# jmg049/Spectrograms

Measured on AMD Instinct MI355X. Metric: STFT frames/sec (f32, n_fft=1024 hop=256), higher is better.
Workload: dtype f32

## Files before the change

### spectrograms_amd/csrc/kernels_r32x16.hip

```cpp
#include <type_traits>
#include <utility>

#include "binaural_kind.h"
#include "buffer_ops.h"
#include "fft_inreg.h"
#include "r32x16_layout.h"
#include "sgx_internal.h"

namespace sgx {
namespace {

using namespace inreg;
using namespace r32x16;

typedef int v4i __attribute__((ext_vector_type(4)));
typedef int v2i __attribute__((ext_vector_type(2)));

__device__ __forceinline__ float db_f32(float x) { return __builtin_log2f(x) * 3.01029995663981195f; }

template <int AMP>
__device__ __forceinline__ float amp_f32(float p, float eps) {
    if constexpr (AMP == AMP_MAGNITUDE) return sqrtf(p);
    else if constexpr (AMP == AMP_DB) return db_f32(fmaxf(p, eps));
    else return p;
// ... 36 lines not shown
#ifndef SGX_ODDHOP
#define SGX_ODDHOP 1
#endif
#ifndef SGX_DMA
#define SGX_DMA 0
#endif
#ifndef SGX_ONEPATH
#define SGX_ONEPATH 1
#endif

template <int OFF>
__device__ __forceinline__ void ds_read64(v2f &d, unsigned addr) {
    asm volatile("ds_read_b64 %0, %1 offset:%2" : "=v"(d) : "v"(addr), "n"(OFF));
}
template <int OFF>
__device__ __forceinline__ void ds_read128(v4f &d, unsigned addr) {
    asm volatile("ds_read_b128 %0, %1 offset:%2" : "=v"(d) : "v"(addr), "n"(OFF));
}
template <int N>
__device__ __forceinline__ void tie8(v2f *d) {
    if constexpr (N >= 0)
        asm volatile("s_waitcnt lgkmcnt(%8)"
                     : "+v"(d[0]), "+v"(d[1]), "+v"(d[2]), "+v"(d[3]), "+v"(d[4]), "+v"(d[5]), "+v"(d[6]), "+v"(d[7])
                     : "n"(N));
    else
        asm volatile("" : "+v"(d[0]), "+v"(d[1]), "+v"(d[2]), "+v"(d[3]), "+v"(d[4]), "+v"(d[5]), "+v"(d[6]), "+v"(d[7]));
}
template <int N>
__device__ __forceinline__ void tie16(v2f (&d)[16]) {
    tie8<N>(&d[0]);
    tie8<-1>(&d[8]);
}
template <bool XSPAD, int N1>
constexpr int col_off() { return N1 * 128 + (XSPAD ? (N1 >> 3) * 128 : 0); }
template <bool XSPAD, int PAR, int... K>
__device__ __forceinline__ void read_cols(v2f (&x)[16], v2f (&w)[16], unsigned xaddr, unsigned waddr, std::integer_sequence<int, K...>) {
    ((ds_read64<col_off<XSPAD, 2 * K + PAR>()>(x[K], xaddr), ds_read64<(2 * K + PAR) * 128>(w[K], waddr)), ...);
}

template <int HOP>
constexpr int p512_off_a(int n1) { return 64 * n1 + (64 * n1 / (8 * HOP)) * 64; }
template <int HOP>
constexpr int p512_off_b(int n1) { return 64 * n1 + 4 * HOP + ((64 * n1 + 4 * HOP) / (8 * HOP)) * 64; }
template <int O0, int O1>
__device__ __forceinline__ void ds_read2x32(v2f &d, unsigned addr) {
    static_assert(O0 >= 0 && O0 < 256 && O1 >= 0 && O1 < 256, "ds_read2_b32: 8-bit dword offsets");
    asm volatile("ds_read2_b32 %0, %1 offset0:%2 offset1:%3" : "=v"(d) : "v"(addr), "n"(O0), "n"(O1));
}
template <int HOP, int PAR, int... K>
__device__ __forceinline__ void read_cols512(v2f (&x)[16], v2f (&w)[16], const unsigned (&base)[8], unsigned waddr, std::integer_sequence<int, K...>) {
    ((ds_read2x32<(p512_off_a<HOP>(2 * K + PAR) - p512_off_a<HOP>((2 * K + PAR) & ~3)) / 4, (p512_off_b<HOP>(2 * K + PAR) - p512_off_a<HOP>((2 * K + PAR) & ~3)) / 4>(
          x[K], base[(2 * K + PAR) >> 2]),
      ds_read64<(2 * K + PAR) * 128>(w[K], waddr)),
     ...);
}

template <int PAR, int... K>
__device__ __forceinline__ void read_cols_odd(v2f (&x)[16], v2f (&w)[16], const unsigned (&base)[4], unsigned waddr, std::integer_sequence<int, K...>) {
    ((ds_read2x32<((2 * K + PAR) & 7) * 32, ((2 * K + PAR) & 7) * 32 + 1>(x[K], base[(2 * K + PAR) >> 3]), ds_read64<(2 * K + PAR) * 128>(w[K], waddr)), ...);
}

template <int PAR, int... K>
__device__ __forceinline__ void read_win(v2f (&w)[16], unsigned waddr, std::integer_sequence<int, K...>) {
    (ds_read64<(2 * K + PAR) * 128>(w[K], waddr), ...);
}

template <int OFF>
__device__ __forceinline__ void dma16_to_lds(__amdgpu_buffer_rsrc_t r, int voff, unsigned lds_base) {
    unsigned keep;
    asm volatile("s_mov_b32 %0, m0\n\ts_mov_b32 m0, %3\n\ts_nop 0\n\tbuffer_load_dwordx4 %1, %2, 0 offen offset:%4 lds\n\ts_mov_b32 m0, %0"
                 : "=&s"(keep)
                 : "v"(voff), "s"(r), "s"(lds_base), "n"(OFF)
                 : "memory");
}
template <bool XSPAD, int R, int ROUNDS>
__device__ __forceinline__ void dma_rounds(__amdgpu_buffer_rsrc_t r, int voff, unsigned xs_base, unsigned wave) {
    if constexpr (R < ROUNDS) {
        const unsigned c0 = R * 256u + wave * 64u;
        dma16_to_lds<0>(r, voff + R * 4096, xs_base + c0 * 16u + (XSPAD ? (c0 >> 6) * 128u : 0u));
        dma_rounds<XSPAD, R + 1, ROUNDS>(r, voff, xs_base, wave);
    }
}

__device__ __forceinline__ void load_tw1(const StftArgs &a, unsigned n2, v2f (&twa)[4], v2f (&twb)[8]) {
    const v2f *t1 = (const v2f *)a.tw1 + n2;
#pragma unroll
    for (int q = 0; q < 4; ++q) twa[q] = t1[16 * 8 * q];
#pragma unroll
    for (int q = 0; q < 8; ++q) twb[q] = t1[16 * q];
}

__device__ __forceinline__ void twiddle_store(v2f (&xr)[32], const v2f (&twa)[4], const v2f (&twb)[8], unsigned char *dst) {
#pragma unroll
    for (int k1 = 0; k1 < 32; ++k1) {
        const int qa = k1 >> 3, qb = k1 & 7;
        v2f r = xr[k1];
        if (qb) r = cmulv(r, twb[qb]);
        if (qa) r = cmulv(r, twa[qa]);
#if defined(SGX_ABL_NOEXW)
        asm volatile("" ::"v"(r), "v"(dst));
#elif defined(SGX_ABL_ADDTID)
        asm volatile("ds_write_addtid_b32 %0 offset:%2\n\tds_write_addtid_b32 %1 offset:%3" ::"v"(r.x), "v"(r.y), "n"(k1 * 512), "n"(k1 * 512 + 256) : "memory");
#else
        *(v2f *)(dst + k1 * 128) = r;
#endif
    }
}

__device__ __forceinline__ void read_rows(const unsigned char *exf, unsigned ra, unsigned rb, v2f (&A)[16], v2f (&B)[16]) {
    const v4f *pa = (const v4f *)(exf + ra * 128);
    const v4f *pb = (const v4f *)(exf + rb * 128);
#pragma unroll
    for (int c = 0; c < 8; ++c) {
        const v4f q = pa[c];
        A[2 * c] = (v2f){q.x, q.y};
        A[2 * c + 1] = (v2f){q.z, q.w};
    }
#pragma unroll
    for (int c = 0; c < 8; ++c) {
        const v4f q = pb[c];
        B[2 * c] = (v2f){q.x, q.y};
        B[2 * c + 1] = (v2f){q.z, q.w};
    }
}

struct JobOfs {
    unsigned a1, b1, a2, b2, mid;
};
__device__ __forceinline__ JobOfs job_offsets(unsigned j, unsigned n_frames) {
    const unsigned c1 = j == 0 ? 16u : j, c2 = j == 0 ? 0u : j + 256u;
    return JobOfs{c1 * n_frames, (512u - 224u - c1) * n_frames, c2 * n_frames, (512u - 224u - c2) * n_frames, 256u * n_frames};
}

struct PwAddr {
    float *up, *down;
};
template <int MODE, int AMP, bool PWT>
__device__ __forceinline__ void pass2_compute(v2f (&A)[16], v2f (&B)[16], bool j0, float eps, const v4f *tw, __amdgpu_buffer_rsrc_t ro,
                                              unsigned oa1, unsigned ob1, unsigned oa2, unsigned ob2, unsigned omid, unsigned step,
                                              float *pw_c1, float *pw_m1, float *pw_c2, float *pw_m2, float *pw_mid SGX_STAMP_PARAMS) {
    Fft<16, false>::run(A, A);
    Fft<16, false>::run(B, B);
    const v2f a8 = A[8];
    if (j0) {
        v2f nA[16], nB[8];
#pragma unroll
        for (int i = 0; i < 8; ++i) { nA[i] = B[i]; nA[8 + i] = A[i]; }
        nB[7] = A[0];
#pragma unroll
        for (int t = 1; t < 8; ++t) nB[7 - t] = A[16 - t];
#pragma unroll
        for (int i = 0; i < 16; ++i) A[i] = nA[i];
#pragma unroll
        for (int i = 0; i < 8; ++i) B[i] = nB[i];
        asm volatile("" ::: "memory");
    }
    SGX_STAMP(9);
    constexpr int PSTEP = MODE == OUT_BINAURAL ? 32 * 16 * 2 : PWT ? 32 * 16 : 32;
    auto emit = [&](unsigned voff, unsigned soff, float *pwp, v2f X, bool conj) {
#ifdef SGX_ABL_NOSTORE
        asm volatile("" ::"v"(X), "v"(voff));
        return;
#endif
        if constexpr (MODE == OUT_COMPLEX) {
            const v2f V = conj ? (v2f){X.x, -X.y} : X;
            __builtin_amdgcn_raw_buffer_store_b64(__builtin_bit_cast(v2i, V), ro, (int)voff, (int)soff, 0);
        } else if constexpr (MODE == OUT_MEL) {
#ifdef SGX_ABL_NOPW
            asm volatile("" ::"v"(X), "v"(pwp));
            return;
#endif
            *pwp = AMP == AMP_MAG_IN ? sqrtf(power_of(X)) : power_of(X);
        } else if constexpr (MODE == OUT_BINAURAL) {
            *(v2f *)pwp = conj ? (v2f){X.x, -X.y} : X;
        } else {
            __builtin_amdgcn_raw_buffer_store_b32(__builtin_bit_cast(int, amp_f32<AMP>(power_of(X), eps)), ro, (int)voff, (int)soff, 0);
        }
    };
    auto split = [&](v2f P, v2f Q, v4f w, v2f &X, v2f &Y) {
        const v2f E = pfma(Q, (v2f){1.f, -1.f}, P);
        const v2f D = pfma(Q, (v2f){-1.f, 1.f}, P);
        const v2f T = pfma(hi2(D), (v2f){w.z, w.w}, lo2(D) * (v2f){w.x, w.y});
        X = E + T;
        Y = E - T;
    };
#pragma unroll
    for (int i = 0; i < 8; ++i) {
        v2f X, Y;
        split(A[i], B[15 - i], tw[i], X, Y);
        emit(oa1, i * step, pw_c1 + i * PSTEP, X, false);
        emit(ob1, (7 - i) * step, pw_m1 + (7 - i) * PSTEP, Y, true);
    }
#pragma unroll
    for (int t = 0; t < 8; ++t) {
        v2f X, Y;
        split(A[8 + t], B[7 - t], tw[8 + t], X, Y);
        emit(oa2, t * step, pw_c2 + t * PSTEP, X, false);
        emit(ob2, (7 - t) * step, pw_m2 + (7 - t) * PSTEP, Y, true);
    }
    if (j0) emit(omid, 0u, pw_mid, a8 * (v2f){2.f, -2.f}, false);
    SGX_STAMP(10);
}

constexpr unsigned kP512Step = 16u * 64u;
template <int MODE, int AMP, bool PACK = false>
__device__ __forceinline__ void pass2_pair512(v2f (&A)[16], v2f (&B)[16], bool j0, float eps, __amdgpu_buffer_rsrc_t ro, unsigned vfull1,
                                              unsigned vhalf1, unsigned vfull2, unsigned vhalf2, unsigned vfullm, unsigned vhalfm, unsigned step,
                                              float *pw1, float *pw2, float *pwm) {
    Fft<16, false>::run(A, A);
    Fft<16, false>::run(B, B);
    const v2f a8 = A[8];
    if (j0) {
        v2f nA[16], nB[8];
#pragma unroll
        for (int i = 0; i < 8; ++i) { nA[i] = B[i]; nA[8 + i] = A[i]; }
        nB[7] = A[0];
#pragma unroll
        for (int t = 1; t < 8; ++t) nB[7 - t] = A[16 - t];
#pragma unroll
        for (int i = 0; i < 16; ++i) A[i] = nA[i];
#pragma unroll
        for (int i = 0; i < 8; ++i) B[i] = nB[i];
        asm volatile("" ::: "memory");
    }
    auto emit = [&](unsigned vfull, unsigned vhalf, int soff, v2f Xa, v2f Xb, bool conj, float *pwp) {
        if constexpr (MODE == OUT_MEL) {
            const float pa = power_of(Xa), pb = power_of(Xb);
            *(v2f *)pwp = AMP == AMP_MAG_IN ? (v2f){sqrtf(pa), sqrtf(pb)} : (v2f){pa, pb};
        } else if constexpr (MODE == OUT_COMPLEX) {
            const float sg = conj ? -1.f : 1.f;
            const v4f V = (v4f){Xa.x, sg * Xa.y, Xb.x, sg * Xb.y};
            if constexpr (PACK) {
                __builtin_amdgcn_raw_buffer_store_b64(__builtin_bit_cast(v2i, (v2f){V.x, V.y}), ro, (int)vfull, soff, 0);
                __builtin_amdgcn_raw_buffer_store_b64(__builtin_bit_cast(v2i, (v2f){V.z, V.w}), ro, (int)vhalf, soff, 0);
            } else {
                __builtin_amdgcn_raw_buffer_store_b128(__builtin_bit_cast(v4i, V), ro, (int)vfull + soff, 0, 0);
                __builtin_amdgcn_raw_buffer_store_b64(__builtin_bit_cast(v2i, (v2f){V.x, V.y}), ro, (int)vhalf, soff, 0);
            }
        } else {
            const v2f V = (v2f){amp_f32<AMP>(power_of(Xa), eps), amp_f32<AMP>(power_of(Xb), eps)};
            if constexpr (PACK) {
                const float va = V.x, vb = V.y;
                __builtin_amdgcn_raw_buffer_store_b32(__builtin_bit_cast(int, va), ro, (int)vfull, soff, 0);
                __builtin_amdgcn_raw_buffer_store_b32(__builtin_bit_cast(int, vb), ro, (int)vhalf, soff, 0);
            } else {
                __builtin_amdgcn_raw_buffer_store_b64(__builtin_bit_cast(v2i, V), ro, (int)vfull, soff, 0);
                __builtin_amdgcn_raw_buffer_store_b32(__builtin_bit_cast(int, V.x), ro, (int)vhalf, soff, 0);
            }
        }
    };
    auto pair = [&](v2f P, v2f Q, v2f &Xa, v2f &Xb) {
        Xa = pfma(Q, (v2f){1.f, -1.f}, P);
        const v2f D = pfma(Q, (v2f){-1.f, 1.f}, P);
        Xb = (v2f){D.y, -D.x};
    };
#pragma unroll
    for (int i = 0; i < 8; ++i) {
        v2f Xa, Xb;
        pair(A[i], B[15 - i], Xa, Xb);
        emit(vfull1, vhalf1, i * (int)step, Xa, Xb, false, pw1 + i * kP512Step);
    }
#pragma unroll
    for (int t = 0; t < 8; ++t) {
        v2f Xa, Xb;
        pair(A[8 + t], B[7 - t], Xa, Xb);
        if (j0) emit(vfull2 + t * step, vhalf2 + t * step, 0, Xa, Xb, false, pw2 + t * kP512Step);
        else emit(vfull2 + (7 - t) * step, vhalf2 + (7 - t) * step, 0, Xa, Xb, true, pw2 + (7 - t) * kP512Step);
    }
    if (j0) emit(vfullm, vhalfm, 0, (v2f){2.f * a8.x, 0.f}, (v2f){2.f * a8.y, 0.f}, false, pwm);
}

template <int AMP>
__device__ __forceinline__ void mel_tile_csr(const StftArgs &a, const float *pwall, unsigned b, unsigned f0, unsigned nf,
                                             float eps, unsigned t, unsigned nthreads) {
    const float *val = (const float *)a.mel_val;
    float *o = (float *)a.out + ((size_t)b * a.n_out) * a.n_frames + f0;
    for (unsigned idx = t; idx < 16u * a.n_mels; idx += nthreads) {
        const unsigned ff = idx & 15u, mm = idx >> 4;
        float acc = 0.0f;
// ... 277 lines not shown
__device__ __forceinline__ void mel_tile_sched512(const StftArgs &a, const float *pwT, const unsigned *sched, unsigned b, unsigned f0,
                                                  unsigned nf, float eps, unsigned tid) {
    const unsigned wave = __builtin_amdgcn_readfirstlane(tid >> 6), lane = tid & 63u, slot = lane >> 4, fp = lane & 15u;
    const unsigned obytes = (a.n_out * a.n_frames - f0) * 4u;
    const __amdgpu_buffer_rsrc_t ro = make_rsrc((const float *)a.out + (size_t)b * a.n_out * a.n_frames + f0, obytes);
    constexpr unsigned kDrop = 0x80000000u;
    const unsigned fo0 = 2u * fp < nf ? 8u * fp : kDrop, fo1 = 2u * fp + 1u < nf ? 8u * fp + 4u : kDrop;
    const uint4 *info = (const uint4 *)(sched + kSchedHdr) + wave * 8u + slot;
    uint4 ca = info[0], cb = info[4];
#pragma unroll
    for (unsigned seg = 0; seg < (unsigned)kSchedSegs; ++seg) {
        const uint4 na = info[(seg + 1u) * 32u], nb = info[(seg + 1u) * 32u + 4u];
        const unsigned L = __builtin_amdgcn_readfirstlane(ca.x);
        const v4f *wa = (const v4f *)((const float *)sched + ca.y), *wb = (const v4f *)((const float *)sched + cb.y);
        const v4f *pa = (const v4f *)(pwT + (ca.z >> 1) * 64u) + fp, *pb = (const v4f *)(pwT + (cb.z >> 1) * 64u) + fp;
        v2f acca = {0.0f, 0.0f}, accb = {0.0f, 0.0f};
        for (unsigned t = 0; t < L; t += 4u) {
            const v4f w4a = wa[t >> 2], a0 = pa[(t >> 1) * 16u], a1 = pa[(t >> 1) * 16u + 16u];
            const v4f w4b = wb[t >> 2], b0 = pb[(t >> 1) * 16u], b1 = pb[(t >> 1) * 16u + 16u];
            acca = mul_add_unfused(w4a.x, (v2f){a0.x, a0.y}, acca);
            accb = mul_add_unfused(w4b.x, (v2f){b0.x, b0.y}, accb);
            acca = mul_add_unfused(w4a.y, (v2f){a0.z, a0.w}, acca);
            accb = mul_add_unfused(w4b.y, (v2f){b0.z, b0.w}, accb);
            acca = mul_add_unfused(w4a.z, (v2f){a1.x, a1.y}, acca);
            accb = mul_add_unfused(w4b.z, (v2f){b1.x, b1.y}, accb);
            acca = mul_add_unfused(w4a.w, (v2f){a1.z, a1.w}, acca);
            accb = mul_add_unfused(w4b.w, (v2f){b1.z, b1.w}, accb);
        }
        const bool ha = ca.w != 0xffffffffu, hb = cb.w != 0xffffffffu;
        const unsigned boa = ca.w * a.n_frames * 4u, bob = cb.w * a.n_frames * 4u;
        __builtin_amdgcn_raw_buffer_store_b32(__builtin_bit_cast(int, amp_f32<AMP>(acca.x, eps)), ro, (int)((ha && fo0 != kDrop) ? boa + fo0 : kDrop), 0, 0);
        __builtin_amdgcn_raw_buffer_store_b32(__builtin_bit_cast(int, amp_f32<AMP>(acca.y, eps)), ro, (int)((ha && fo1 != kDrop) ? boa + fo1 : kDrop), 0, 0);
        __builtin_amdgcn_raw_buffer_store_b32(__builtin_bit_cast(int, amp_f32<AMP>(accb.x, eps)), ro, (int)((hb && fo0 != kDrop) ? bob + fo0 : kDrop), 0, 0);
        __builtin_amdgcn_raw_buffer_store_b32(__builtin_bit_cast(int, amp_f32<AMP>(accb.y, eps)), ro, (int)((hb && fo1 != kDrop) ? bob + fo1 : kDrop), 0, 0);
        ca = na;
        cb = nb;
    }
}

template <int KIND>
__device__ __forceinline__ void binaural_tile(const StftArgs &a, const unsigned char *smem_all, unsigned b, unsigned f0, unsigned nf) {
    binaural::KindConst<float> c;
    c.pi = 3.14159265358979323846f;
    c.two_pi = 2.0f * c.pi;
    c.bw = (float)a.bin_bw;
    c.power = a.bin_power;
    c.wrapped = a.bin_wrapped;
    const v2f *L = (const v2f *)smem_all, *R = (const v2f *)(smem_all + kExBytes);
    float *out = (float *)a.out + ((size_t)b * a.bin_count) * a.n_frames + f0;
    for (unsigned i = threadIdx.x; i < a.bin_count * 16u; i += 512u) {
        const unsigned r = i >> 4, f = i & 15u, k = a.bin_start + r;
        const v2f l = L[k * 16u + f], q = R[k * 16u + f];
        const float v = binaural::binaural_value<float, KIND>(l.x, l.y, q.x, q.y, k, c);
        if (f < nf) out[(size_t)r * a.n_frames + f] = v;
    }
}

template <int MODE, int AMP, int ROUNDS, bool WIDE, bool XSPAD, bool PWT, int HOP512 = 0, bool PACK = false, int MSTEPS = 0>
__global__ __launch_bounds__(512, 2) void k_r32x16(StftArgs a, unsigned per_xcd, unsigned total, unsigned slots) {
    constexpr bool MFCC = MSTEPS != 0;
    static_assert(!MFCC || (PWT && AMP == AMP_DB && HOP512 == 0 && !PACK), "fused MFCC epilogue: Mel-dB on the schedule, n_fft 1024, one-signal tiles");
    constexpr bool P512 = HOP512 != 0;
    constexpr bool BIN = MODE == OUT_BINAURAL;
    static_assert(!BIN || (!WIDE && !PWT && !P512 && !PACK && !MFCC), "binaural: one-signal n_fft 1024 tiles, per-half pass 2");
    constexpr unsigned HS = BIN ? 1u : 2u;
    static_assert(!PACK || (ROUNDS == 0 && !WIDE && !XSPAD && (HOP512 == 0 ? (MODE != OUT_MEL || PWT) : MODE != OUT_MEL)),
                  "PACK: direct loads, one-half tiles; n_fft 1024: scheduled band stage, n_fft 512: per-bin outputs");
    constexpr unsigned SS512 = 8u * HOP512;
    static_assert(!P512 || PACK || (HOP512 % 4 == 0 && ROUNDS * 256 * 4 >= 31 * HOP512 + 512), "P512: 16-byte chunks, the whole tile staged");
    static_assert(!WIDE || MODE != OUT_MEL, "wide pass 2 needs a per-bin output");
    static_assert(!PWT || MODE == OUT_MEL, "PWT is a filterbank layout");
    static_assert(!P512 || (!WIDE && !XSPAD && (ROUNDS > 0 || PACK) && (PWT == (MODE == OUT_MEL))), "P512: staged samples (PACK: per-lane loads), scheduled band stage");
    constexpr bool DMA = SGX_DMA != 0 && PWT && ROUNDS > 0 && !P512;
    constexpr unsigned FPT = P512 ? 32u : 16u;
    constexpr unsigned NB = P512 ? 257u : 513u;
    extern __shared__ __attribute__((aligned(16))) unsigned char smem_all[];
    const unsigned half = __builtin_amdgcn_readfirstlane(threadIdx.x >> 8);
    const unsigned tid = threadIdx.x & 255u;
    constexpr bool H256M = HOP512 == 256 && MODE == OUT_MEL && !PACK;
    constexpr unsigned EXB = H256M ? (unsigned)kExBytesH256 : (unsigned)kExBytes, POFF = H256M ? (unsigned)kOutOffH256 : (unsigned)kOutOff;
    unsigned char *smem = smem_all + half * EXB;
    unsigned char *tabs = smem_all + 2 * EXB;
    if (threadIdx.x < 256u) ((v4f *)(tabs + kWinOff))[threadIdx.x] = ((const v4f *)a.window)[threadIdx.x];
    for (unsigned i = threadIdx.x; i < 16u * 17u; i += 512u) ((v4f *)(tabs + kTw2Off))[i] = ((const v4f *)a.tw2)[i];
    unsigned *sched = (unsigned *)(tabs + kMelOff);
    if constexpr (PWT)
        for (unsigned i = threadIdx.x; i < a.mel_sched_words; i += 512u) sched[i] = a.mel_sched[i];
    float *mfrag = (float *)(tabs + kMelOff) + ((a.mel_sched_words + 3u) & ~3u);
    if constexpr (MFCC)
        for (unsigned i = threadIdx.x; i < a.mfcc_frag_words; i += 512u) mfrag[i] = ((const float *)a.mfcc_frag)[i];

    const unsigned xcd = blockIdx.x & 7u, slot = blockIdx.x >> 3;
    const unsigned lo = xcd * per_xcd;
    const unsigned hi = min(lo + per_xcd, total);
    unsigned wid = lo + slot * HS + (BIN ? 0u : half);
    unsigned lead = lo + slot * HS;

    const unsigned p1f = tid >> 4, n2 = tid & 15u;
    const unsigned lane = tid & 63u;
    const unsigned wv_ = WIDE ? threadIdx.x >> 6 : tid >> 6;
    const unsigned jq = WIDE ? lane >> 5 : lane >> 4, p2f = WIDE ? lane & 31u : lane & 15u;
    const unsigned j = wv_ + (WIDE ? 8u : 4u) * jq;
    const unsigned ra = j, rb = j == 0 ? 16u : 32u - j;
    const float eps = (float)a.eps;
    constexpr unsigned ES = MODE == OUT_COMPLEX ? 8u : 4u;
    const JobOfs jo = job_offsets(j, a.n_frames);
    const unsigned step = 32u * a.n_frames * ES;
    const v4f *twj = (const v4f *)(tabs + kTw2Off) + j * 17u;
    v2f twa[4], twb[8];
    load_tw1(a, n2, twa, twb);

    constexpr int NCR = ROUNDS > 0 ? ROUNDS : 1;
    v4f creg[NCR];
    v2f xd[ROUNDS > 0 ? 1 : 32];
    const unsigned chunks = XSPAD ? 1216u : P512 ? (31u * HOP512 + 512u + 3u) >> 2 : (15u * a.hop + 1024u + 3u) >> 2;
    const unsigned hop = XSPAD ? 256u : (P512 && !PACK) ? (unsigned)HOP512 : a.hop;
    const unsigned row_bytes = (unsigned)a.n_samples * 4u;
    auto load_tile = [&](unsigned w) {
        const unsigned b = w / a.tiles, tile = w - b * a.tiles;
        const unsigned f0 = tile * FPT;
        const __amdgpu_buffer_rsrc_t rx = make_rsrc((const float *)(BIN && half ? a.x2 : a.x) + (size_t)b * a.sample_stride, row_bytes);
        const int tile_lo = (int)(f0 * hop) - (int)a.pad;
        const bool interior = tile_lo >= 0 && (unsigned)tile_lo + (FPT - 1u) * hop + (P512 ? 512u : 1024u) <= (unsigned)a.n_samples;
        if constexpr (ROUNDS > 0) {
#ifdef SGX_ABL_NOGLOAD
            for (int r = 0; r < ROUNDS; ++r) creg[r] = (v4f){(float)w, 1.f, 2.f, (float)r};
            return;
#endif
            const int vo = (tile_lo + 4 * (int)tid) * 4;
            if constexpr (DMA) {
                dma_rounds<XSPAD, 0, ROUNDS>(rx, vo, lds_addr(smem), __builtin_amdgcn_readfirstlane(tid >> 6));
                return;
            }
            if (SGX_ONEPATH || interior || P512) {
#pragma unroll
                for (int r = 0; r < ROUNDS; ++r)
                    if (SGX_ONEPATH || XSPAD || P512 || r * 256u + tid < chunks) creg[r] = __builtin_bit_cast(v4f, __builtin_amdgcn_raw_buffer_load_b128(rx, vo + r * 4096, 0, 0));
            } else {
#pragma unroll
                for (int r = 0; r < ROUNDS; ++r) {
                    v4i c;
#pragma unroll
                    for (int e = 0; e < 4; ++e) c[e] = __builtin_amdgcn_raw_buffer_load_b32(rx, vo + r * 4096 + 4 * e, 0, 0);
                    creg[r] = __builtin_bit_cast(v4f, c);
                }
            }
        } else if constexpr (PACK && P512) {
            const __amdgpu_buffer_rsrc_t rall = make_rsrc(a.x, a.x_bytes);
            const unsigned ns = (unsigned)a.n_samples, PP = (a.n_frames + 1u) >> 1;
            const unsigned q = w * 16u + p1f;
            const bool live = q < a.gframes;
            const unsigned bq = live ? q / PP : 0u, pr = q - bq * PP;
            const int sA = (int)(2u * pr * hop) - (int)a.pad + (int)n2, sB = sA + (int)hop;
            const unsigned row = bq * (unsigned)a.sample_stride;
#pragma unroll
            for (int n1 = 0; n1 < 32; ++n1) {
                const int ia = sA + 16 * n1, ib = sB + 16 * n1;
                const int va = __builtin_amdgcn_raw_buffer_load_b32(rall, (live && (unsigned)ia < ns) ? (int)((row + (unsigned)ia) * 4u) : (int)0xfffffff0u, 0, 0);
                const int vb = __builtin_amdgcn_raw_buffer_load_b32(rall, (live && (unsigned)ib < ns) ? (int)((row + (unsigned)ib) * 4u) : (int)0xfffffff0u, 0, 0);
                xd[n1] = (v2f){__builtin_bit_cast(float, va), __builtin_bit_cast(float, vb)};
            }
        } else if constexpr (PACK) {
            const unsigned g = w * 16u + p1f;
            const bool live = g < a.gframes;
            const unsigned bq = live ? g / a.n_frames : 0u, fq = g - bq * a.n_frames;
            const __amdgpu_buffer_rsrc_t rall = make_rsrc(a.x, a.x_bytes);
            const int s0 = (int)(fq * hop) - (int)a.pad + 2 * (int)n2;
            const unsigned rowo = bq * (unsigned)a.sample_stride;
            const unsigned ns = (unsigned)a.n_samples;
#pragma unroll
            for (int n1 = 0; n1 < 32; ++n1) {
                const int sidx = s0 + 32 * n1;
                const bool in0 = live && (unsigned)sidx < ns;
                v2f v = __builtin_bit_cast(v2f, __builtin_amdgcn_raw_buffer_load_b64(rall, in0 ? (int)((rowo + (unsigned)sidx) * 4u) : (int)0xfffffff0u, 0, 0));
                if ((unsigned)(sidx + 1) >= ns) v.y = 0.0f;
                xd[n1] = v;
            }
        } else {
            const int vo = ((int)(p1f * hop) + tile_lo + 2 * (int)n2) * 4;
            if (SGX_ONEPATH || interior) {
#pragma unroll
                for (int n1 = 0; n1 < 32; ++n1) xd[n1] = __builtin_bit_cast(v2f, __builtin_amdgcn_raw_buffer_load_b64(rx, vo + n1 * 128, 0, 0));
#if SGX_ODDHOP
                if (a.hop & 1u) {
                    const float x0 = __builtin_bit_cast(float, __builtin_amdgcn_raw_buffer_load_b32(rx, 0, 0, 0));
                    const int s0 = (int)(p1f * hop) + tile_lo + 2 * (int)n2;
#pragma unroll
                    for (int n1 = 0; n1 < 32; ++n1)
                        if (s0 + 32 * n1 == -1) xd[n1].y = x0;
                }
#endif
            } else {
#pragma unroll
// ... 39 lines not shown
    static_assert(!MFCC || kOutOff - 256 * mfcc_row<MFCC ? MSTEPS : 4>() >= 22912, "Mel-dB tile above the staged samples");
    while (lead < hi) {
        const unsigned PP = (a.n_frames + 1u) >> 1;
        const unsigned b = PACK ? (P512 ? wid * 16u / PP : wid * 16u / a.n_frames) : wid / a.tiles, tile = wid - b * a.tiles;
        const unsigned f0 = PACK ? wid * 16u - b * a.n_frames : tile * FPT;
        const unsigned nf = PACK ? min(16u, a.gframes - wid * 16u) : min(FPT, a.n_frames - f0);
        v2f xr[32];
        {
            v2f e[16], o[16], we[16], wo[16];
            if constexpr (ROUNDS > 0) {
                if constexpr (DMA) {
                    asm volatile("s_waitcnt vmcnt(%0)" ::"n"(2 * kSchedSegs) : "memory");
                } else {
#pragma unroll
                for (int r = 0; r < ROUNDS; ++r) {
                    const unsigned c = r * 256u + tid;
                    if (SGX_ONEPATH || XSPAD || P512 || c < chunks) *(v4f *)(smem + c * 16u + (XSPAD ? (c >> 6) * 128u : P512 ? (c * 16u / (P512 ? SS512 : 1u)) * 64u : 0u)) = creg[r];
                }
                }
                SGX_STAMP(0);
                __syncthreads();
                SGX_STAMP(1);
                if constexpr (MFCC) mfcc_tile<MFCC ? MSTEPS : 4>(a, mfl, mfrag, mfcc_mt, pvb, pvf0, pvnf, tid & 63u);
                if constexpr (HOP512 == 256) {
                    const float *pa = (const float *)(smem + p1f * (SS512 + 64u) + n2 * 4u);
#pragma unroll
                    for (int k = 0; k < 16; ++k) {
                        e[k] = (v2f){pa[p512_off_a<256>(2 * k) / 4], pa[p512_off_b<256>(2 * k) / 4]};
                        o[k] = (v2f){pa[p512_off_a<256>(2 * k + 1) / 4], pa[p512_off_b<256>(2 * k + 1) / 4]};
                    }
                    read_win<0>(we, waddr, std::make_integer_sequence<int, 16>{});
                    read_win<1>(wo, waddr, std::make_integer_sequence<int, 16>{});
                    tie16<0>(e);
                    tie16<-1>(o);
                    tie16<-1>(we);
                    tie16<-1>(wo);
                } else if constexpr (P512) {
                    unsigned base[8];
#pragma unroll
                    for (int q = 0; q < 8; ++q) base[q] = lds_addr(smem) + p1f * (SS512 + 64u) + n2 * 4u + (unsigned)p512_off_a<P512 ? HOP512 : 128>(4 * q);
                    read_cols512<P512 ? HOP512 : 128, 0>(e, we, base, waddr, std::make_integer_sequence<int, 16>{});
                    read_cols512<P512 ? HOP512 : 128, 1>(o, wo, base, waddr, std::make_integer_sequence<int, 16>{});
                    tie16<15>(e);
                    tie16<-1>(we);
                } else {
                if (SGX_ODDHOP && !XSPAD && (a.hop & 1u)) {
                    const unsigned base[4] = {xaddr, xaddr + 1024u, xaddr + 2048u, xaddr + 3072u};
                    read_cols_odd<0>(e, we, base, waddr, std::make_integer_sequence<int, 16>{});
                    read_cols_odd<1>(o, wo, base, waddr, std::make_integer_sequence<int, 16>{});
                } else {
                read_cols<XSPAD, 0>(e, we, xaddr, waddr, std::make_integer_sequence<int, 16>{});
                read_cols<XSPAD, 1>(o, wo, xaddr, waddr, std::make_integer_sequence<int, 16>{});
                }
                tie16<15>(e);
                tie16<-1>(we);
                }
            } else {
                const v2f *w2 = (const v2f *)(tabs + kWinOff) + n2;
#pragma unroll
                for (int k = 0; k < 16; ++k) {
                    e[k] = xd[2 * k];
                    o[k] = xd[2 * k + 1];
                    we[k] = w2[32 * k];
                    wo[k] = w2[32 * k + 16];
                }
            }
            Fft<16, true>::run(e, we);
            if constexpr (ROUNDS > 0) {
                tie16<0>(o);
                tie16<-1>(wo);
            }
            Fft<16, true>::run(o, wo);
            Comb<32, 0, v2f>::run(xr, e, o);
        }
        SGX_STAMP(2);
        if constexpr (ROUNDS > 0 || MFCC) __syncthreads();
        SGX_STAMP(3);
#ifdef SGX_ABL_ADDTID
        {
            const unsigned m0v = __builtin_amdgcn_readfirstlane(lds_addr(smem) + (tid >> 6) * 16384u);
            asm volatile("s_mov_b32 m0, %0\n\ts_nop 0" ::"s"(m0v) : "memory");
        }
#endif
        twiddle_store(xr, twa, twb, smem + p1f * kFS + n2 * 8);
        SGX_STAMP(4);
        unsigned next = lead + slots * HS + (BIN ? 0u : half);
        if (next >= hi) next -= BIN ? 0u : half;
        if constexpr (!DMA)
            if (lead + slots * HS < hi) load_tile(next);
        SGX_STAMP(5);
        __syncthreads();
        SGX_STAMP(6);
        constexpr bool ALLSTORE = MODE != OUT_MEL;
        unsigned p2b = b, p2ofs, p2ex;
        if constexpr (WIDE) {
            const unsigned w1 = lead + 1u < hi ? lead + 1u : lead;
            const unsigned b0 = lead / a.tiles, f00 = (lead - b0 * a.tiles) * 16u;
            const unsigned b1 = w1 / a.tiles, f01 = (w1 - b1 * a.tiles) * 16u;
            const unsigned nf0 = min(16u, a.n_frames - f00), nf1 = min(16u, a.n_frames - f01);
            const bool second = p2f >= 16u && w1 != lead;
            const unsigned fle = min(p2f & 15u, (second ? nf1 : nf0) - 1u);
            p2ex = (second ? 16u : 0u) + fle;
            p2ofs = (second ? f01 : f00) + fle + ((second && b1 != b0) ? 513u * a.n_frames : 0u);
            p2b = b0;
        } else if constexpr (P512) {
            p2ex = p2f;
            p2ofs = f0 + 2u * p2f;
        } else if constexpr (PACK) {
            const unsigned p2f_eff = ALLSTORE ? min(p2f, nf - 1u) : p2f;
            const unsigned fl = f0 + p2f_eff, bq = fl / a.n_frames;
            p2ex = p2f_eff;
            p2ofs = bq * NB * a.n_frames + (fl - bq * a.n_frames);
        } else {
            const unsigned p2f_eff = ALLSTORE ? min(p2f, nf - 1u) : p2f;
            p2ex = p2f_eff;
            p2ofs = f0 + p2f_eff;
        }
        v2f A[16], B[16];
        read_rows((WIDE ? smem_all : smem) + p2ex * kFS, ra, rb, A, B);
        SGX_STAMP(7);
        __syncthreads();
        SGX_STAMP(8);
        if constexpr (DMA)
            if (lead + slots * HS < hi) load_tile(next);
        float *pwf = (float *)(smem + (PWT ? POFF : 0u));
        if constexpr (MODE == OUT_MEL) {
            if constexpr (P512) {
                for (unsigned i = tid; i < 11u * 32u; i += 256u) pwf[pwt512_index(257u + (i >> 5), i & 31u)] = 0.0f;
            } else if constexpr (PWT) {
                if (tid < 176u) pwf[pwt_index(513u + (tid >> 4), tid & 15u)] = 0.0f;
            } else {
                if (tid < 48u) pwf[(tid / 3u) * kPS + 513u + tid % 3u] = 0.0f;
            }
        }
        if constexpr (BIN) {
            const unsigned c1 = j == 0 ? 16u : j, c2 = j == 0 ? 0u : j + 256u;
            auto slot_of = [&](unsigned k) { return (float *)smem + (k * 16u + p2f) * 2u; };
            pass2_compute<MODE, AMP, false>(A, B, j == 0, eps, twj, make_rsrc(a.out, 0u), 0u, 0u, 0u, 0u, 0u, 0u, slot_of(c1),
                                            slot_of(512u - 224u - c1), slot_of(c2), slot_of(512u - 224u - c2), slot_of(256u) SGX_STAMP_ARGS);
            __syncthreads();
            binaural_tile<AMP>(a, smem_all, b, f0, nf);
            __syncthreads();
        } else if constexpr (P512 && PACK) {
            constexpr unsigned kDrop = 0x80000000u;
            const __amdgpu_buffer_rsrc_t ro = make_rsrc((unsigned char *)a.out + (size_t)b * NB * a.n_frames * ES, min(17u, a.batch - b) * NB * a.n_frames * ES);
            const unsigned c1 = j == 0 ? 16u : j, r2 = j == 0 ? 0u : 32u - j;
            const unsigned q = wid * 16u + p2f, bq = q / PP, pr = q - bq * PP;
            const unsigned oA = p2f < nf ? ((bq - b) * NB * a.n_frames + 2u * pr) * ES : kDrop;
            const unsigned oB = (p2f < nf && 2u * pr + 1u < a.n_frames) ? oA + ES : kDrop;
            auto at = [&](unsigned base, unsigned row) { return base == kDrop ? kDrop : base + row * a.n_frames * ES; };
            pass2_pair512<MODE, AMP, true>(A, B, j == 0, eps, ro, at(oA, c1), at(oB, c1), at(oA, r2), at(oB, r2), at(oA, 256u), at(oB, 256u), step,
                                           nullptr, nullptr, nullptr);
        } else if constexpr (P512) {
            constexpr unsigned kDrop = 0x80000000u;
            const __amdgpu_buffer_rsrc_t ro = make_rsrc((unsigned char *)a.out + (size_t)b * NB * a.n_frames * ES, NB * a.n_frames * ES);
            const unsigned c1 = j == 0 ? 16u : j, r2 = j == 0 ? 0u : 32u - j;
            const unsigned nv = 2u * p2f + 1u < nf ? 2u : 2u * p2f < nf ? 1u : 0u;
            const unsigned o1 = (c1 * a.n_frames + p2ofs) * ES, o2 = (r2 * a.n_frames + p2ofs) * ES, om = (256u * a.n_frames + p2ofs) * ES;
            float *pws = pwf + 4u * p2f;
            pass2_pair512<MODE, AMP>(A, B, j == 0, eps, ro, nv == 2u ? o1 : kDrop, nv == 1u ? o1 : kDrop, nv == 2u ? o2 : kDrop,
                                     nv == 1u ? o2 : kDrop, nv == 2u ? om : kDrop, nv == 1u ? om : kDrop, step, pws + pwt512_index(c1, 0u),
                                     pws + pwt512_index(r2, 0u), pws + pwt512_index(256u, 0u));
        } else if (ALLSTORE || p2f < nf) {
            const unsigned c1 = j == 0 ? 16u : j, c2 = j == 0 ? 0u : j + 256u;
            const unsigned long long obytes = (unsigned long long)min(PACK ? 17u : 2u, a.batch - p2b) * 513ull * a.n_frames * ES;
            const __amdgpu_buffer_rsrc_t ro = make_rsrc((unsigned char *)a.out + (size_t)p2b * 513u * a.n_frames * ES, (unsigned)obytes);
            {
                auto slot_of = [&](unsigned k) { return pwf + (PWT ? pwt_index(k, p2f) : p2f * kPS + k); };
                pass2_compute<MODE, AMP, PWT>(A, B, j == 0, eps, twj, ro, (jo.a1 + p2ofs) * ES, (jo.b1 + p2ofs) * ES, (jo.a2 + p2ofs) * ES,
                                                     (jo.b2 + p2ofs) * ES, (jo.mid + p2ofs) * ES, step, slot_of(c1), slot_of(512u - 224u - c1),
                                                     slot_of(c2), slot_of(512u - 224u - c2), slot_of(256u) SGX_STAMP_ARGS);
            }
        }
        if constexpr (MODE == OUT_MEL) {
            __syncthreads();
            SGX_STAMP(11);
#ifdef SGX_ABL_NOMEL
            if (a.n_mels == 12345u)
#endif
            if constexpr (P512) mel_tile_sched512<AMP>(a, pwf, sched, b, f0, nf, eps, tid);
            else if constexpr (MFCC) {
                mel_tile_sched<AMP, false, mfcc_row<MFCC ? MSTEPS : 4>()>(a, pwf, sched, b, f0, nf, eps, tid, mfl SGX_STAMP_ARGS);
                if constexpr (ROUNDS > 0) {
                    pvb = b; pvf0 = f0; pvnf = nf;
                } else {
                    __syncthreads();
                    mfcc_tile<MFCC ? MSTEPS : 4>(a, mfl, mfrag, mfcc_mt, b, f0, nf, tid & 63u);
                }
            }
            else if constexpr (PWT) mel_tile_sched<AMP, PACK>(a, pwf, sched, b, f0, nf, eps, tid, nullptr SGX_STAMP_ARGS);
            else if (a.mm_frag) map_tile_mfma<AMP>(a, pwf, b, f0, nf, eps, tid, 2u * half);
            else mel_tile_csr<AMP>(a, pwf, b, f0, nf, eps, tid, 256u);
            if constexpr (!PWT) __syncthreads();
        }
        SGX_STAMP(14);
        wid = next;
        lead += slots * HS;
#ifdef SGX_STAMPS
        st_acc[15] += 1;
#endif
    }
    if constexpr (MFCC && ROUNDS > 0) {
        __syncthreads();
        mfcc_tile<MFCC ? MSTEPS : 4>(a, mfl, mfrag, mfcc_mt, pvb, pvf0, pvnf, tid & 63u);
    }
#ifdef SGX_SKEW
    if (MODE == OUT_MEL && half == 0u)
        for (unsigned q = 0; q < SGX_SKEW; ++q) __syncthreads();
#endif
#ifdef SGX_STAMPS
    if ((threadIdx.x & 63u) == 0) {
        for (int q = 0; q < 16; ++q) atomicAdd(&g_stamps[q], st_acc[q]);
        atomicAdd(&g_stamps[16], 1ull);
    }
#endif
}

static bool want_pack(const StftArgs &a, bool mel, bool pwt) {
    if (a.mfcc_frag) return false;
    const bool p512 = a.n_fft == 512u;
    const bool unlisted512 = p512 && !(a.hop == 64u || a.hop == 128u || a.hop == 160u || a.hop == 256u);
    if ((a.n_fft != 1024u && !p512) || (a.batch < 2u && !unlisted512) || (mel && (!pwt || p512)) || (a.hop & 1u)) return false;
    const unsigned long long slots = (unsigned long long)a.tiles * a.ft, g = (unsigned long long)a.batch * a.n_frames;
    const unsigned long long used = p512 ? 2ull * ((a.n_frames + 1ull) / 2ull) : a.n_frames;
    if ((slots - used) * 4ull < slots && !unlisted512) return false;
    if (g >= 0x7fffffffull || (unsigned long long)a.batch * a.sample_stride * 4ull >= 0xfffffff0ull) return false;
    return (a.ft + 1ull) * (a.n_fft / 2u + 1ull) * a.n_frames * 8ull < 0x7fffffffull;
}

template <int MODE, int AMP>
hipError_t launch_variant(const StftArgs &a0, hipStream_t s) {
    StftArgs a = a0;
    const bool pack = want_pack(a, MODE == OUT_MEL, MODE == OUT_MEL && a.mel_sched != nullptr);
    const bool pack512 = pack && a.n_fft == 512u;
    a.gframes = pack512 ? a.batch * ((a.n_frames + 1u) / 2u) : a.batch * a.n_frames;
    a.x_bytes = pack ? (unsigned)((unsigned long long)a.batch * a.sample_stride * 4ull) : 0u;
    const unsigned total = pack ? (a.gframes + 15u) / 16u : a.tiles * a.batch;
    const unsigned per_xcd = (total + 7) / 8;
    const unsigned chunks = (15u * a.hop + 1024u + 3u) >> 2;
    const unsigned pairs = (per_xcd + 1) / 2;
#ifndef SGX_SLOTS
#define SGX_SLOTS 0u
#endif
    const unsigned cu_slots = SGX_SLOTS ? SGX_SLOTS : std::max(1u, device_cu_count() / 8u);
    const unsigned nslots = pairs < cu_slots ? pairs : cu_slots;
    const bool pwt = MODE == OUT_MEL && a.mel_sched != nullptr;
    auto go = [&](auto kernel, unsigned lds = (unsigned)kLdsBytes) -> hipError_t {
        hipError_t e = set_max_dynamic_lds((const void *)kernel, 163840);
        if (e != hipSuccess) return e;
        hipLaunchKernelGGL(kernel, dim3(nslots * 8), dim3(512), lds, s, a, per_xcd, total, nslots);
        return hipGetLastError();
    };
// ... 135 lines not shown
```

### spectrograms_amd/csrc/r32x16_layout.h

```cpp
#pragma once

namespace sgx {
namespace r32x16 {

constexpr int kFS = 4096 + 16;
constexpr int kPS = 516;
constexpr int kExBytes = 16 * kFS;
constexpr int kOutOff = kExBytes - 16 * 17 * 128;
constexpr int kWinOff = 0;
constexpr int kTw2Off = 4096;
constexpr int kTw2Bytes = 16 * 17 * 16;
constexpr int kMelOff = kTw2Off + kTw2Bytes;
constexpr int kMelMaxWords = 4096;
constexpr int kLdsBytes = 2 * kExBytes + kMelOff + kMelMaxWords * 4;
constexpr int kExBytesH256 = 72960;
constexpr int kOutOffH256 = kExBytesH256 - 16 * 17 * 128;
constexpr int kMelMaxWordsH256 = (163840 - 2 * kExBytesH256 - kMelOff) / 4 - 16;

constexpr int kSchedHdr = 4;
constexpr int kSchedSegs = 4;

}

namespace r32x32 {
constexpr int kFS2 = 8192 + 16;
constexpr int kEx2 = 16 * kFS2;
constexpr int kPw2Off = kEx2 - 518 * 128;
constexpr int kWin2Off = 0;
constexpr int kTw22Off = 8192;
constexpr int kSch2Off = kTw22Off + 32 * 17 * 16;
constexpr int kLds2Base = kEx2 + kSch2Off;
constexpr int kLds2Max = 163840;
constexpr int kSch2MaxWords = (kLds2Max - kLds2Base - 64) / 4;
constexpr int kSegs2 = 3;
}
}
```

Baseline: 1.416 billion.

## Move inter-pass twiddles from pass-1 store to pass-2 row multiply with packed FMA

For non-mel, non-512 paths, the 1024-point STFT's twiddle multiplication moves out of the pass-1 twiddle_store, which now keeps only a single rotation on element 0. Pass 2 instead multiplies each row by per-row twiddles (conjugated for the mirrored row) right after reading them from LDS. The split twiddle table is repacked into a compact half-size layout, and row twiddles are staged in LDS. Complex multiplies use hand-written v_pk_fma_f32 with op_sel/neg modifiers to save instructions. This reorganizes the j==0 reindexing (ROT) and changes LDS table layout, risking correctness and register pressure.

```diff
diff --git a/spectrograms_amd/csrc/kernels_r32x16.hip b/spectrograms_amd/csrc/kernels_r32x16.hip
--- a/spectrograms_amd/csrc/kernels_r32x16.hip
+++ b/spectrograms_amd/csrc/kernels_r32x16.hip
@@ -142,6 +142,21 @@
     }
 }
 
+template <bool CONJ>
+__device__ __forceinline__ v2f cmul_reg(v2f x, v2f t) {
+    const v2f c = x * lo2(t);
+    v2f r;
+    if constexpr (CONJ) asm("v_pk_fma_f32 %0, %1, %2, %3 op_sel:[1,1,0] op_sel_hi:[0,1,1] neg_hi:[0,1,0]" : "=v"(r) : "v"(x), "v"(t), "v"(c));
+    else asm("v_pk_fma_f32 %0, %1, %2, %3 op_sel:[1,1,0] op_sel_hi:[0,1,1] neg_lo:[0,1,0]" : "=v"(r) : "v"(x), "v"(t), "v"(c));
+    return r;
+}
+__device__ __forceinline__ v2f split_tw(v2f D, v2f w) {
+    const v2f c = lo2(D) * w;
+    v2f r;
+    asm("v_pk_fma_f32 %0, %1, %2, %3 op_sel:[1,1,0] op_sel_hi:[1,0,1] neg_lo:[0,1,0]" : "=v"(r) : "v"(D), "v"(w), "v"(c));
+    return r;
+}
+
 __device__ __forceinline__ void load_tw1(const StftArgs &a, unsigned n2, v2f (&twa)[4], v2f (&twb)[8]) {
     const v2f *t1 = (const v2f *)a.tw1 + n2;
 #pragma unroll
@@ -150,13 +165,18 @@
     for (int q = 0; q < 8; ++q) twb[q] = t1[16 * q];
 }
 
+template <bool P2>
 __device__ __forceinline__ void twiddle_store(v2f (&xr)[32], const v2f (&twa)[4], const v2f (&twb)[8], unsigned char *dst) {
 #pragma unroll
     for (int k1 = 0; k1 < 32; ++k1) {
         const int qa = k1 >> 3, qb = k1 & 7;
         v2f r = xr[k1];
-        if (qb) r = cmulv(r, twb[qb]);
-        if (qa) r = cmulv(r, twa[qa]);
+        if constexpr (P2) {
+            if (k1 == 0) r = cmul_reg<true>(r, twa[2]);
+        } else {
+            if (qb) r = cmulv(r, twb[qb]);
+            if (qa) r = cmulv(r, twa[qa]);
+        }
 #if defined(SGX_ABL_NOEXW)
         asm volatile("" ::"v"(r), "v"(dst));
 #elif defined(SGX_ABL_ADDTID)
@@ -192,27 +212,50 @@
     return JobOfs{c1 * n_frames, (512u - 224u - c1) * n_frames, c2 * n_frames, (512u - 224u - c2) * n_frames, 256u * n_frames};
 }
 
+__device__ __forceinline__ void pass2_twiddle(v2f (&A)[16], v2f (&B)[16], const v2f (&t)[16]) {
+#pragma unroll
+    for (int n = 1; n < 16; ++n) {
+        A[n] = cmul_reg<false>(A[n], t[n]);
+        B[n] = cmul_reg<true>(B[n], t[n]);
+    }
+}
+
 struct PwAddr {
     float *up, *down;
 };
-template <int MODE, int AMP, bool PWT>
+template <int MODE, int AMP, bool PWT, bool ROT>
 __device__ __forceinline__ void pass2_compute(v2f (&A)[16], v2f (&B)[16], bool j0, float eps, const v4f *tw, __amdgpu_buffer_rsrc_t ro,
                                               unsigned oa1, unsigned ob1, unsigned oa2, unsigned ob2, unsigned omid, unsigned step,
                                               float *pw_c1, float *pw_m1, float *pw_c2, float *pw_m2, float *pw_mid SGX_STAMP_PARAMS) {
+    constexpr int R = ROT ? 1 : 0;
     Fft<16, false>::run(A, A);
     Fft<16, false>::run(B, B);
-    const v2f a8 = A[8];
+    const v2f a8 = ROT ? B[9] : A[8];
     if (j0) {
-        v2f nA[16], nB[8];
-#pragma unroll
-        for (int i = 0; i < 8; ++i) { nA[i] = B[i]; nA[8 + i] = A[i]; }
-        nB[7] = A[0];
-#pragma unroll
-        for (int t = 1; t < 8; ++t) nB[7 - t] = A[16 - t];
-#pragma unroll
-        for (int i = 0; i < 16; ++i) A[i] = nA[i];
-#pragma unroll
-        for (int i = 0; i < 8; ++i) B[i] = nB[i];
+        if constexpr (ROT) {
+            v2f nA[8], nB[16];
+#pragma unroll
+            for (int t = 0; t < 8; ++t) nA[t] = B[t + 1];
+#pragma unroll
+            for (int i = 0; i < 8; ++i) nB[(16 - i) & 15] = A[15 - i];
+#pragma unroll
+            for (int t = 0; t < 8; ++t) nB[8 - t] = B[(17 - t) & 15];
+#pragma unroll
+            for (int t = 0; t < 8; ++t) A[8 + t] = nA[t];
+#pragma unroll
+            for (int i = 0; i < 16; ++i) B[i] = nB[i];
+        } else {
+            v2f nA[16], nB[8];
+#pragma unroll
+            for (int i = 0; i < 8; ++i) { nA[i] = B[i]; nA[8 + i] = A[i]; }
+            nB[7] = A[0];
+#pragma unroll
+            for (int t = 1; t < 8; ++t) nB[7 - t] = A[16 - t];
+#pragma unroll
+            for (int i = 0; i < 16; ++i) A[i] = nA[i];
+#pragma unroll
+            for (int i = 0; i < 8; ++i) B[i] = nB[i];
+        }
         asm volatile("" ::: "memory");
     }
     SGX_STAMP(9);
@@ -237,24 +280,28 @@
             __builtin_amdgcn_raw_buffer_store_b32(__builtin_bit_cast(int, amp_f32<AMP>(power_of(X), eps)), ro, (int)voff, (int)soff, 0);
         }
     };
-    auto split = [&](v2f P, v2f Q, v4f w, v2f &X, v2f &Y) {
+    auto twi = [&](int i) {
+        const v4f q = tw[i >> 1];
+        return (i & 1) ? (v2f){q.z, q.w} : (v2f){q.x, q.y};
+    };
+    auto split = [&](v2f P, v2f Q, v2f w, v2f &X, v2f &Y) {
         const v2f E = pfma(Q, (v2f){1.f, -1.f}, P);
         const v2f D = pfma(Q, (v2f){-1.f, 1.f}, P);
-        const v2f T = pfma(hi2(D), (v2f){w.z, w.w}, lo2(D) * (v2f){w.x, w.y});
+        const v2f T = split_tw(D, w);
         X = E + T;
         Y = E - T;
     };
 #pragma unroll
     for (int i = 0; i < 8; ++i) {
         v2f X, Y;
-        split(A[i], B[15 - i], tw[i], X, Y);
+        split(A[i], B[(15 + R - i) & 15], twi(i), X, Y);
         emit(oa1, i * step, pw_c1 + i * PSTEP, X, false);
         emit(ob1, (7 - i) * step, pw_m1 + (7 - i) * PSTEP, Y, true);
     }
 #pragma unroll
     for (int t = 0; t < 8; ++t) {
         v2f X, Y;
-        split(A[8 + t], B[7 - t], tw[8 + t], X, Y);
+        split(A[8 + t], B[7 + R - t], twi(8 + t), X, Y);
         emit(oa2, t * step, pw_c2 + t * PSTEP, X, false);
         emit(ob2, (7 - t) * step, pw_m2 + (7 - t) * PSTEP, Y, true);
     }
@@ -698,7 +745,12 @@
     unsigned char *smem = smem_all + half * EXB;
     unsigned char *tabs = smem_all + 2 * EXB;
     if (threadIdx.x < 256u) ((v4f *)(tabs + kWinOff))[threadIdx.x] = ((const v4f *)a.window)[threadIdx.x];
-    for (unsigned i = threadIdx.x; i < 16u * 17u; i += 512u) ((v4f *)(tabs + kTw2Off))[i] = ((const v4f *)a.tw2)[i];
+    if (threadIdx.x < 256u) {
+        const unsigned jj = threadIdx.x >> 4, ii = threadIdx.x & 15u;
+        const v4f q = ((const v4f *)a.tw2)[jj * 17u + ii];
+        *(v2f *)(tabs + kTw2Off + jj * kTw2Stride + ii * 8u) = (v2f){q.x, q.y};
+        *(v2f *)(tabs + kTrOff + jj * 128u + ii * 8u) = ((const v2f *)a.tw1)[(jj == 0u ? 16u : jj) * 16u + ii];
+    }
     unsigned *sched = (unsigned *)(tabs + kMelOff);
     if constexpr (PWT)
         for (unsigned i = threadIdx.x; i < a.mel_sched_words; i += 512u) sched[i] = a.mel_sched[i];
@@ -717,14 +769,23 @@
     const unsigned wv_ = WIDE ? threadIdx.x >> 6 : tid >> 6;
     const unsigned jq = WIDE ? lane >> 5 : lane >> 4, p2f = WIDE ? lane & 31u : lane & 15u;
     const unsigned j = wv_ + (WIDE ? 8u : 4u) * jq;
-    const unsigned ra = j, rb = j == 0 ? 16u : 32u - j;
+    constexpr bool TWP2 = !P512 && MODE != OUT_MEL;
+    constexpr bool TRLDS = TWP2 && ROUNDS == 0 && !WIDE;
+    const unsigned ra = j == 0 ? (TWP2 ? 16u : 0u) : j, rb = j == 0 ? (TWP2 ? 0u : 16u) : 32u - j;
     const float eps = (float)a.eps;
     constexpr unsigned ES = MODE == OUT_COMPLEX ? 8u : 4u;
     const JobOfs jo = job_offsets(j, a.n_frames);
     const unsigned step = 32u * a.n_frames * ES;
-    const v4f *twj = (const v4f *)(tabs + kTw2Off) + j * 17u;
-    v2f twa[4], twb[8];
-    load_tw1(a, n2, twa, twb);
+    const v4f *twj = (const v4f *)(tabs + kTw2Off + j * kTw2Stride);
+    v2f twa[4], twb[8], tr[16];
+    if constexpr (!TWP2) {
+        load_tw1(a, n2, twa, twb);
+    } else {
+        twa[2] = ((const v2f *)a.tw1)[16 * 16 + n2];
+        if constexpr (!TRLDS)
+#pragma unroll
+            for (int q = 0; q < 16; ++q) tr[q] = ((const v2f *)a.tw1)[ra * 16u + q];
+    }
 
     constexpr int NCR = ROUNDS > 0 ? ROUNDS : 1;
     v4f creg[NCR];
@@ -930,7 +991,7 @@
             asm volatile("s_mov_b32 m0, %0\n\ts_nop 0" ::"s"(m0v) : "memory");
         }
 #endif
-        twiddle_store(xr, twa, twb, smem + p1f * kFS + n2 * 8);
+        twiddle_store<TWP2>(xr, twa, twb, smem + p1f * kFS + n2 * 8);
         SGX_STAMP(4);
         unsigned next = lead + slots * HS + (BIN ? 0u : half);
         if (next >= hi) next -= BIN ? 0u : half;
@@ -966,6 +1027,16 @@
         }
         v2f A[16], B[16];
         read_rows((WIDE ? smem_all : smem) + p2ex * kFS, ra, rb, A, B);
+        if constexpr (TRLDS) {
+            const v4f *tq = (const v4f *)(tabs + kTrOff + j * 128u);
+#pragma unroll
+            for (int q = 0; q < 8; ++q) {
+                const v4f t2 = tq[q];
+                tr[2 * q] = (v2f){t2.x, t2.y};
+                tr[2 * q + 1] = (v2f){t2.z, t2.w};
+            }
+        }
+        if constexpr (TWP2) pass2_twiddle(A, B, tr);
         SGX_STAMP(7);
         __syncthreads();
         SGX_STAMP(8);
@@ -984,7 +1055,7 @@
         if constexpr (BIN) {
             const unsigned c1 = j == 0 ? 16u : j, c2 = j == 0 ? 0u : j + 256u;
             auto slot_of = [&](unsigned k) { return (float *)smem + (k * 16u + p2f) * 2u; };
-            pass2_compute<MODE, AMP, false>(A, B, j == 0, eps, twj, make_rsrc(a.out, 0u), 0u, 0u, 0u, 0u, 0u, 0u, slot_of(c1),
+            pass2_compute<MODE, AMP, false, TWP2>(A, B, j == 0, eps, twj, make_rsrc(a.out, 0u), 0u, 0u, 0u, 0u, 0u, 0u, slot_of(c1),
                                             slot_of(512u - 224u - c1), slot_of(c2), slot_of(512u - 224u - c2), slot_of(256u) SGX_STAMP_ARGS);
             __syncthreads();
             binaural_tile<AMP>(a, smem_all, b, f0, nf);
@@ -1015,7 +1086,7 @@
             const __amdgpu_buffer_rsrc_t ro = make_rsrc((unsigned char *)a.out + (size_t)p2b * 513u * a.n_frames * ES, (unsigned)obytes);
             {
                 auto slot_of = [&](unsigned k) { return pwf + (PWT ? pwt_index(k, p2f) : p2f * kPS + k); };
-                pass2_compute<MODE, AMP, PWT>(A, B, j == 0, eps, twj, ro, (jo.a1 + p2ofs) * ES, (jo.b1 + p2ofs) * ES, (jo.a2 + p2ofs) * ES,
+                pass2_compute<MODE, AMP, PWT, TWP2>(A, B, j == 0, eps, twj, ro, (jo.a1 + p2ofs) * ES, (jo.b1 + p2ofs) * ES, (jo.a2 + p2ofs) * ES,
                                                      (jo.b2 + p2ofs) * ES, (jo.mid + p2ofs) * ES, step, slot_of(c1), slot_of(512u - 224u - c1),
                                                      slot_of(c2), slot_of(512u - 224u - c2), slot_of(256u) SGX_STAMP_ARGS);
             }
diff --git a/spectrograms_amd/csrc/r32x16_layout.h b/spectrograms_amd/csrc/r32x16_layout.h
--- a/spectrograms_amd/csrc/r32x16_layout.h
+++ b/spectrograms_amd/csrc/r32x16_layout.h
@@ -9,7 +9,10 @@
 constexpr int kOutOff = kExBytes - 16 * 17 * 128;
 constexpr int kWinOff = 0;
 constexpr int kTw2Off = 4096;
+constexpr int kTw2Stride = 144;
 constexpr int kTw2Bytes = 16 * 17 * 16;
+constexpr int kTrOff = kTw2Off + 16 * kTw2Stride;
+static_assert(kTrOff + 16 * 128 <= kTw2Off + kTw2Bytes, "row twiddles inside the table area");
 constexpr int kMelOff = kTw2Off + kTw2Bytes;
 constexpr int kMelMaxWords = 4096;
 constexpr int kLdsBytes = 2 * kExBytes + kMelOff + kMelMaxWords * 4;
```

Measured after the change: 1.458 billion (median of 6 runs). +3.0%, better.
